# isi-vista/VistaOCR

Measured on AMD Instinct MI355X. Metric: line-images/sec (train, batch 32, 30x600 grey), higher is better.
Workload: dtype f32 (the LSTM's large GEMMs as bf16x6 products: fp32 operands split exactly into three bf16 planes, six bf16 MFMAs per fp32 product, fp32 accumulate; VOCR_LSTM_GEMM=f32 restores the f32-MFMA kernels); 1 GPU; configs[1]: 32 synthetic 1x30x600 grey lines per GPU, 20 labels/line, V=96, 3xBiLSTM-512, train() = H2D of the batch + fwd+CTC+bwd+allreduce+clamp+Adam, loss returned as a float; widths=600 .. 600 px, mean 600, conv_dtype=fp32, global_batch=32, parallelism=dp1, ranks_seen=1, backend=none, per_rank_rng=seed 1234 + 1000*rank after an identical init

## Files before the change

### include/vocr.h

```cpp
#ifndef VOCR_H
#define VOCR_H
#include <stddef.h>
#include <stdint.h>

#ifdef __cplusplus
extern "C" {
#endif

#define VOCR_OK          0
#define VOCR_EINVAL     -1
#define VOCR_ELAUNCH    -2
#define VOCR_ENODEVICE  -3
#define VOCR_ECOMM      -4


const char* vocr_last_error(void);
#define VOCR_ABI_VERSION 5
int  vocr_abi_version(void);
int  vocr_profile_range_push(const char* name);
int  vocr_profile_range_pop(void);
int  vocr_device_count(void);

int vocr_conv3x3_pack_weights(const float* w, float* wpack_fwd, float* wpack_dgrad, int cout, int cin, void* stream);
int vocr_conv3x3_fwd(const float* x, const float* wpack, const float* bias, float* y,
// ... 22 lines not shown
int vocr_conv3x3_wgrad_f16(const float* x, const float* dy, float* dw, void* workspace,
                           int n, int cin, int h, int w, int cout, void* stream);
int vocr_conv3x3_h16_supported(int cin, int cout);
int vocr_conv3x3_h16_plan(int n, int cin, int h, int w, int cout);
int vocr_conv3x3_h16_fwd(const void* x16, const void* wpack, const float* bias, float* y,
                         int n, int cin, int h, int w, int cout, void* stream);
int vocr_f16_padded_row(int w);
int vocr_f32_to_f16_layouts(const float* x, void* nhwc, void* nchwp, int n, int c, int h, int w, void* stream);
int vocr_conv3x3_wgrad_h16_supported(int cin, int cout);
size_t vocr_conv3x3_wgrad_h16_workspace_bytes(int n, int cin, int h, int w, int cout);
int vocr_conv3x3_wgrad_h16(const void* x16p, const void* dy16p, float* dw, void* workspace,
                           int n, int cin, int h, int w, int cout, void* stream);
size_t vocr_channel_sum_workspace_bytes(int n, int c, int hw);
int vocr_channel_sum(const float* x, float* out, int n, int c, int hw, void* workspace, void* stream);

size_t vocr_bn_workspace_bytes(int n, int c, int hw);
int vocr_bn_train_stats(const float* y, int n, int c, int hw, float eps, float momentum,
                        float* mean, float* invstd, float* running_mean, float* running_var,
                        int64_t* num_batches_tracked, float* xhat_sum, void* workspace, void* stream);
int vocr_bn_eval_stats(const float* running_mean, const float* running_var, int c, float eps,
                       float* mean, float* invstd, void* stream);
int vocr_bn_relu_apply(const float* y, const float* mean, const float* invstd, const float* gamma,
                       const float* beta, float* out, int n, int c, int hw, void* stream);
int vocr_bn_train_relu_apply(const float* y, const float* gamma, const float* beta, float* out, int n, int c, int hw, float eps,
                             float momentum, float* mean, float* invstd, float* running_mean, float* running_var,
                             int64_t* num_batches_tracked, float* xhat_sum, void* workspace, void* stream);
int vocr_bn_train_relu_fracpool2x2_fwd(const float* y, const float* gamma, const float* beta, const float* samples, float* out,
                                       int32_t* idx, int n, int c, int h, int w, int oh, int ow, float eps, float momentum,
                                       float* mean, float* invstd, float* running_mean, float* running_var,
                                       int64_t* num_batches_tracked, float* xhat_sum, void* workspace, void* stream);
int vocr_bn_relu_bwd(const float* da, const float* y, const float* mean, const float* invstd,
                     const float* gamma, const float* beta, const float* xhat_sum, float* dy, float* dgamma, float* dbeta,
                     float* dconv_bias, int n, int c, int hw, void* workspace, void* stream);

int vocr_fracpool2x2_fwd(const float* x, const float* samples, float* out, int32_t* idx,
                         int n, int c, int h, int w, int oh, int ow, void* stream);
int vocr_bn_relu_fracpool2x2_fwd(const float* y, const float* mean, const float* invstd, const float* gamma,
                                 const float* beta, const float* samples, float* out, int32_t* idx,
                                 int n, int c, int h, int w, int oh, int ow, void* stream);
int vocr_bn_relu_fracpool2x2_bwd_supported(int h, int w, int oh, int ow);
int vocr_bn_relu_fracpool2x2_bwd(const float* dout, const int32_t* idx, const float* samples, const float* y,
                                 const float* mean, const float* invstd, const float* gamma, const float* beta,
                                 const float* xhat_sum, float* dy, float* dgamma, float* dbeta, float* dconv_bias,
                                 int n, int c, int h, int w, int oh, int ow, void* workspace, void* stream);
int vocr_fracpool2x2_bwd(const float* dout, const int32_t* idx, float* dx,
                         int n, int c, int h, int w, int oh, int ow, void* stream);

int vocr_relu_maxpool2_fwd(const float* x, float* out, int32_t* idx, int n, int c, int h, int w, void* stream);
int vocr_relu_maxpool2_bwd(const float* dout, const float* out, const int32_t* idx, float* dx,
                           int n, int c, int h, int w, void* stream);

size_t vocr_gemm_workspace_bytes(int m, int n, int k, int has_bias_or_relu);
int vocr_gemm(int transa, int transb, int m, int n, int k,
              const float* a, int lda, const float* b, int ldb, float* c, int ldc,
              const float* bias, int relu, int accumulate, void* workspace, size_t workspace_bytes, void* stream);
#define VOCR_GEMM_PLAN_INTS 12
int vocr_gemm_plan(int transa, int transb, int m, int n, int k, int lda, int ldb, int ldc, int aligned, int has_bias_or_relu,
                   int accumulate, size_t workspace_bytes, int nprob, int nseg, int tiles_only, int* plan);
size_t vocr_gemm_pair_workspace_bytes(int m, int n, int k, int mode);
int vocr_gemm_pair(int mode, int transa, int transb, int m, int n, int k, const float* a0, const float* a1, int lda,
                   const float* b0, const float* b1, int ldb, float* c0, float* c1, int ldc, const float* bias0, const float* bias1,
                   int relu, void* workspace, size_t workspace_bytes, void* stream);
size_t vocr_colsum_workspace_bytes(int m, int n);
int vocr_colsum(const float* x, float* out, int m, int n, void* workspace, void* stream);
int vocr_relu_bwd(const float* dy, const float* out, float* dz, size_t count, void* stream);
int vocr_bchw_to_wbch(const float* x, float* out, int b, int c, int h, int w, void* stream);
// ... 172 lines not shown
```

### vistaocr_amd/_lib.py

```python
import ctypes
import os
from ctypes import c_char_p, c_float, c_int, c_size_t, c_uint32, c_uint64, c_void_p

_HERE = os.path.dirname(os.path.abspath(__file__))
LIB_PATH = os.path.join(_HERE, "csrc", "libvocr.so")

P, I, F, Z, U64, U32 = c_void_p, c_int, c_float, c_size_t, c_uint64, c_uint32

SIGNATURES = {
    "vocr_last_error": (c_char_p, []),
    "vocr_abi_version": (I, []),
    "vocr_device_count": (I, []),
    "vocr_profile_range_push": (I, [c_char_p]),
    "vocr_profile_range_pop": (I, []),
    "vocr_conv3x3_pack_weights": (I, [P, P, P, I, I, P]),
    "vocr_conv3x3_fwd": (I, [P, P, P, P, I, I, I, I, I, P]),
    "vocr_conv3x3_wgrad_workspace_bytes": (Z, [I, I, I, I, I]),
    "vocr_conv3x3_wgrad": (I, [P, P, P, P, I, I, I, I, I, P]),
    "vocr_conv3x3_wino_supported": (I, [I, I]),
    "vocr_conv3x3_wino_pack_floats": (Z, [I, I]),
    "vocr_conv3x3_wino_pack_weights": (I, [P, P, P, I, I, P]),
    "vocr_conv3x3_wino_fwd": (I, [P, P, P, P, I, I, I, I, I, P]),
    "vocr_conv3x3_wino_plan": (I, [I, I, I, I, I]),
    "vocr_conv3x3_wgrad_wino_workspace_bytes": (Z, [I, I, I, I, I]),
    "vocr_conv3x3_wgrad_wino": (I, [P, P, P, P, I, I, I, I, I, P]),
    "vocr_conv3x3_f16_pack_bytes": (Z, [I, I, I]),
    "vocr_conv3x3_f16_pack_weights": (I, [P, P, P, I, I, P]),
    "vocr_conv3x3_f16_fwd": (I, [P, P, P, P, I, I, I, I, I, P]),
    "vocr_conv3x3_wgrad_f16": (I, [P, P, P, P, I, I, I, I, I, P]),
    "vocr_conv3x3_c1_fwd": (I, [P, P, P, P, I, I, I, I, I, P]),
    "vocr_conv3x3_c1_wgrad_workspace_bytes": (Z, [I, I, I]),
    "vocr_conv3x3_c1_wgrad": (I, [P, P, P, P, P, I, I, I, I, P]),
    "vocr_conv3x3_h16_supported": (I, [I, I]),
    "vocr_conv3x3_h16_plan": (I, [I, I, I, I, I]),
    "vocr_conv3x3_h16_fwd": (I, [P, P, P, P, I, I, I, I, I, P]),
    "vocr_f16_padded_row": (I, [I]),
    "vocr_f32_to_f16_layouts": (I, [P, P, P, I, I, I, I, P]),
    "vocr_conv3x3_wgrad_h16_supported": (I, [I, I]),
    "vocr_conv3x3_wgrad_h16_workspace_bytes": (Z, [I, I, I, I, I]),
    "vocr_conv3x3_wgrad_h16": (I, [P, P, P, P, I, I, I, I, I, P]),
    "vocr_channel_sum_workspace_bytes": (Z, [I, I, I]),
    "vocr_channel_sum": (I, [P, P, I, I, I, P, P]),
    "vocr_bn_workspace_bytes": (Z, [I, I, I]),
    "vocr_bn_train_stats": (I, [P, I, I, I, F, F, P, P, P, P, P, P, P, P]),
    "vocr_bn_eval_stats": (I, [P, P, I, F, P, P, P]),
    "vocr_bn_relu_apply": (I, [P, P, P, P, P, P, I, I, I, P]),
    "vocr_bn_train_relu_apply": (I, [P, P, P, P, I, I, I, F, F, P, P, P, P, P, P, P, P]),
    "vocr_bn_train_relu_fracpool2x2_fwd": (I, [P, P, P, P, P, P, I, I, I, I, I, I, F, F, P, P, P, P, P, P, P, P]),
    "vocr_bn_relu_bwd": (I, [P, P, P, P, P, P, P, P, P, P, P, I, I, I, P, P]),
    "vocr_bn_relu_fracpool2x2_bwd_supported": (I, [I, I, I, I]),
    "vocr_bn_relu_fracpool2x2_bwd": (I, [P] * 13 + [I] * 6 + [P, P]),
    "vocr_fracpool2x2_fwd": (I, [P, P, P, P, I, I, I, I, I, I, P]),
    "vocr_bn_relu_fracpool2x2_fwd": (I, [P, P, P, P, P, P, P, P, I, I, I, I, I, I, P]),
    "vocr_fracpool2x2_bwd": (I, [P, P, P, I, I, I, I, I, I, P]),
    "vocr_relu_maxpool2_fwd": (I, [P, P, P, I, I, I, I, P]),
    "vocr_relu_maxpool2_bwd": (I, [P, P, P, P, I, I, I, I, P]),
    "vocr_gemm_workspace_bytes": (Z, [I, I, I, I]),
    "vocr_gemm": (I, [I, I, I, I, I, P, I, P, I, P, I, P, I, I, P, Z, P]),
    "vocr_gemm_plan": (I, [I, I, I, I, I, I, I, I, I, I, I, Z, I, I, I, P]),
    "vocr_gemm_pair_workspace_bytes": (Z, [I, I, I, I]),
    "vocr_gemm_pair": (I, [I, I, I, I, I, I, P, P, I, P, P, I, P, P, I, P, P, I, P, Z, P]),
    "vocr_gemm_x6_planes_bytes": (Z, [I, I]),
    "vocr_gemm_x6_split": (I, [P, P, I, I, P, ctypes.c_long, I, I, I, P, P]),
    "vocr_gemm_x6_workspace_bytes": (Z, [I, I, I]),
    "vocr_gemm_x6_plan": (I, [I, I, I, I, I, I, I, P]),
    "vocr_gemm_x6": (I, [P, I, I, I, I, P, I, I, I, I, I, I, I, P, P, I, I, I, P, P, I, P, P]),
    "vocr_gemm_x6_two_views": (I, [P, I, I, I, P, I, I, I, I, I, I, I, I, I, I, I, I, P, P, I, P, P]),
    "vocr_gemm_h3_two_views": (I, [P, I, I, I, P, I, I, I, I, I, I, I, I, I, I, I, I, P, P, I, P, P]),
    "vocr_gemm_h3_planes_bytes": (Z, [I, I]),
    "vocr_gemm_h3_split": (I, [P, P, I, I, P, ctypes.c_long, I, I, I, ctypes.c_float, P, P]),
    "vocr_gemm_h3": (I, [P, I, I, I, I, P, I, I, I, I, I, I, I, P, P, I, I, I, P, P, I, P, P]),
    "vocr_colsum_workspace_bytes": (Z, [I, I]),
    "vocr_colsum": (I, [P, P, I, I, P, P]),
    "vocr_relu_bwd": (I, [P, P, P, Z, P]),
    "vocr_bchw_to_wbch": (I, [P, P, I, I, I, I, P]),
    "vocr_wbch_to_bchw": (I, [P, P, I, I, I, I, P]),
    "vocr_mul": (I, [P, P, P, Z, P]),
    "vocr_add": (I, [P, P, P, Z, P]),
    "vocr_scale_dev": (I, [P, P, P, Z, P]),
    "vocr_dropout_fwd": (I, [P, P, P, Z, F, U64, P]),
    "vocr_dropout_mask": (I, [P, Z, F, U64, P]),
    "vocr_lstm_workspace_bytes": (Z, [I, I, I]),
# ... 138 lines not shown
```

### vistaocr_amd/build.py

```python
import hashlib
import json
import os
import shutil
import subprocess
import sys
from concurrent.futures import ThreadPoolExecutor

CSRC = os.path.join(os.path.dirname(os.path.abspath(__file__)), "csrc")
SOURCES = ["gemm.hip", "gemm_dma.hip", "gemm_x6.hip", "conv.hip", "conv_wino.hip", "conv_f16.hip", "bn_pool.hip", "lstm.hip", "ctc.hip", "ctc_beam.hip", "ctc_word_beam.hip", "ctc_align.hip", "ctc_edit.hip", "ctc_nbest.hip", "ctc_entropy.hip", "ctc_keyword.hip", "ctc_grammar.hip", "ctc_grammar_beam.hip", "edit_distance.hip", "augment.hip", "misc.cpp", "comm.cpp"]
HEADERS = [os.path.join(CSRC, "vocr_common.h"), os.path.join(CSRC, "conv_tail.h"), os.path.join(CSRC, "gemm_dma.h"),
           os.path.join(CSRC, "ctc_math.h"), os.path.join(CSRC, "ctc_beam_common.h"), os.path.join(CSRC, "ctc_align_common.h"),
           os.path.join(CSRC, "ctc_lattice.h"),
           os.path.join(CSRC, "..", "..", "include", "vocr.h")]
LIB = os.path.join(CSRC, "libvocr.so")
STAMP = os.path.join(CSRC, "build", "libvocr.stamp")
ARCH = "gfx950"
FLAGS = ["-O3", "--offload-arch=" + ARCH, "-fPIC", "-std=c++17", "-Wno-pass-failed"]
_REPORT = {"built": False, "reason": "not asked"}


def _hipcc():
    for cand in (shutil.which("hipcc"), "/opt/rocm/bin/hipcc"):
        if cand and os.path.exists(cand):
            return cand
    return None


def _tree_hash():
    h = hashlib.sha256()
    for path in [os.path.join(CSRC, s) for s in SOURCES] + HEADERS:
        h.update(os.path.basename(path).encode() + b"\0")
        with open(path, "rb") as f:
            h.update(f.read())
    h.update(" ".join(FLAGS).encode())
    return h.hexdigest()


def tree_hash():
    return _tree_hash()


def _compiler_id(hipcc):
    if not hipcc:
# ... 90 lines not shown
```

### vistaocr_amd/csrc/bn_pool.hip

```cpp
#include "vocr_common.h"

namespace {

constexpr int BN_CHUNK_ELEMS = 16384;

__host__ __device__ inline int bn_nchunk(long per_channel) {
    long n = (per_channel + BN_CHUNK_ELEMS - 1) / BN_CHUNK_ELEMS;
    return (int)(n < 1 ? 1 : (n > 512 ? 512 : n));
}

__device__ __forceinline__ long chan_addr(long e, int c, int C, long HW) {
    const long n = e / HW, r = e - n * HW;
    return (n * C + c) * HW + r;
}

struct ChanWalk {
    long n;
    long r;
    __device__ __forceinline__ ChanWalk(long e, long HW) : n(e / HW), r(e - (e / HW) * HW) {}
    __device__ __forceinline__ long addr(int c, int C, long HW) const { return (n * C + c) * HW + r; }
    __device__ __forceinline__ void advance(long step, long HW) {
        r += step;
        while (r >= HW) { r -= HW; ++n; }
    }
};

__device__ __forceinline__ void block_reduce2(double& a, double& b, double* red) {
    a = wave_sum_d(a);
    b = wave_sum_d(b);
    const int wave = threadIdx.x >> 6;
    if ((threadIdx.x & 63) == 0) { red[wave * 2] = a; red[wave * 2 + 1] = b; }
    __syncthreads();
    a = (red[0] + red[2]) + (red[4] + red[6]);
// ... 806 lines not shown
        pool_bwd_lds_kernel<8192><<<(unsigned)(n * c), 512, 0, s>>>(dout, idx, dx, (int)in_plane, oh * ow);
    } else if (use_lds && in_plane <= 18432) {
        pool_bwd_lds_kernel<18432><<<(unsigned)(n * c), 512, 0, s>>>(dout, idx, dx, (int)in_plane, oh * ow);
    } else if (use_lds && in_plane <= 36864) {
        pool_bwd_lds_kernel<36864><<<(unsigned)(n * c), 512, 0, s>>>(dout, idx, dx, (int)in_plane, oh * ow);
    } else {
        if (hipMemsetAsync(dx, 0, (size_t)n * c * in_plane * sizeof(float), s) != hipSuccess) {
            vocr_set_error("vocr_fracpool2x2_bwd: memset failed");
            return VOCR_ELAUNCH;
        }
        pool_bwd_scatter_kernel<<<plane_grid((long)n * c, (long)oh * ow), 256, 0, s>>>(dout, idx, dx, in_plane, oh * ow);
    }
    VOCR_CHECK_LAUNCH("vocr_fracpool2x2_bwd");
    return VOCR_OK;
}

extern "C" int vocr_relu_maxpool2_fwd(const float* x, float* out, int32_t* idx, int n, int c, int h, int w, void* stream) {
    VOCR_CHECK_ARG(x && out && idx && n > 0 && c > 0 && h >= 2 && w >= 2 && (long)n * c <= 65535, "vocr_relu_maxpool2_fwd: bad argument");
    const int oh = h / 2, ow = w / 2;
    relu_maxpool2_fwd_kernel<<<plane_grid((long)n * c, (long)oh * ow), 256, 0, (hipStream_t)stream>>>(x, out, idx, h, w, oh, ow);
    VOCR_CHECK_LAUNCH("vocr_relu_maxpool2_fwd");
    return VOCR_OK;
}

extern "C" int vocr_relu_maxpool2_bwd(const float* dout, const float* out, const int32_t* idx, float* dx, int n, int c,
                                      int h, int w, void* stream) {
    VOCR_CHECK_ARG(dout && out && idx && dx && n > 0 && c > 0 && (long)n * c <= 65535, "vocr_relu_maxpool2_bwd: bad argument");
    const int oh = h / 2, ow = w / 2;
    relu_maxpool2_bwd_kernel<<<plane_grid((long)n * c, (long)oh * ow), 256, 0, (hipStream_t)stream>>>(dout, out, idx, dx,
                                                                                                  (long)h * w, oh * ow);
    VOCR_CHECK_LAUNCH("vocr_relu_maxpool2_bwd");
    return VOCR_OK;
}
```

### vistaocr_amd/csrc/conv.hip

```cpp
#include "vocr_common.h"
#include "conv_tail.h"

namespace {

constexpr int SEGW = 32;
constexpr int CI_C = 8;
constexpr int KC = CI_C * 9;
constexpr int PROW = SEGW + 2;
constexpr int PCI = 3 * PROW;
constexpr int PSEG = CI_C * PCI;

__global__ void pack_weights_kernel(const float* __restrict__ w, float* __restrict__ pf, float* __restrict__ pd,
                                    int cout, int cin) {
    const int i = blockIdx.x * blockDim.x + threadIdx.x;
    const int total = cout * cin * 9;
    if (i >= total) return;
    const int tap = i % 9, ci = (i / 9) % cin, co = i / (9 * cin);
    const float v = w[i];
    if (pf) pf[(long)(ci * 9 + tap) * cout + co] = v;
    if (pd) pd[(long)(co * 9 + (8 - tap)) * cin + ci] = v;
}

struct SegGeom { int FS, RW, RR, per_img, nseg; };

__host__ __device__ inline SegGeom seg_geom(int N, int H, int W) {
    SegGeom g;
    g.FS = W / SEGW;
    g.RW = W % SEGW;
    g.RR = g.RW ? (PROW / (g.RW + 2)) : 1;
    if (g.RR > H) g.RR = H;
    g.per_img = H * g.FS + (g.RW ? (H + g.RR - 1) / g.RR : 0);
    g.nseg = N * g.per_img;
    return g;
}
// ... 1270 lines not shown
    const int QW = (W + 3) >> 2;
    const int q = blockIdx.x * 256 + threadIdx.x;
    if (q >= H * QW) return;
    const int h = q / QW, w0 = (q % QW) * 4;
    const float* xi = x + (long)n * H * W;
    float win[3][6];
#pragma unroll
    for (int kh = 0; kh < 3; ++kh) {
        const int hh = h + kh - 1;
        const bool rok = hh >= 0 && hh < H;
        const float* row = xi + (long)(rok ? hh : 0) * W;
#pragma unroll
        for (int j = 0; j < 6; ++j) {
            const int ww = w0 - 1 + j;
            float v = (rok && ww >= 0 && ww < W) ? row[ww] : 0.f;
            if (round_f16) v = (float)(_Float16)v;
            win[kh][j] = v;
        }
    }
    float* yo = y + ((long)n * Cout * H + h) * W + w0;
    const long cstride = (long)H * W;
    const bool full = w0 + 3 < W && ((((uintptr_t)yo) | ((uintptr_t)(cstride * 4))) & 15) == 0;
    for (int co = 0; co < Cout; ++co) {
        float k[9];
#pragma unroll
        for (int t = 0; t < 9; ++t) {
            k[t] = w[co * 9 + t];
            if (round_f16) k[t] = (float)(_Float16)k[t];
        }
        const float b = bias ? bias[co] : 0.f;
        float o[4];
#pragma unroll
        for (int p = 0; p < 4; ++p) {
            float a = 0.f;
#pragma unroll
            for (int kh = 0; kh < 3; ++kh)
#pragma unroll
                for (int kw = 0; kw < 3; ++kw) a = __builtin_fmaf(win[kh][p + kw], k[kh * 3 + kw], a);
            o[p] = a + b;
        }
        float* d = yo + co * cstride;
        if (full) {
            *(f32x4*)d = (f32x4){o[0], o[1], o[2], o[3]};
        } else {
#pragma unroll
            for (int p = 0; p < 4; ++p)
                if (w0 + p < W) d[p] = o[p];
        }
    }
}

__global__ __launch_bounds__(256) void conv3x3_c1_wgrad_kernel(const float* __restrict__ x, const float* __restrict__ dy,
                                                               float* __restrict__ part, int N, int H, int W, int Cout, int rows_per_split) {
    __shared__ float red[40][257];
    const int tid = threadIdx.x;
    const int cg = blockIdx.x, split = blockIdx.y;
    const int co0 = cg * 4;
    const int nco = min(4, Cout - co0);
    const long HW = (long)H * W;
    const int r0 = split * rows_per_split, r1 = min(N * H, r0 + rows_per_split);
    float acc[4][10];
#pragma unroll
    for (int c = 0; c < 4; ++c)
#pragma unroll
        for (int t = 0; t < 10; ++t) acc[c][t] = 0.f;
    const int QW = (W + 3) >> 2;
    const bool vec = (W & 3) == 0 && ((((uintptr_t)x) | ((uintptr_t)dy)) & 15) == 0;
    for (long q = (long)r0 * QW + tid; q < (long)r1 * QW; q += 256) {
        const int r = (int)(q / QW), w0 = (int)(q % QW) * 4;
        const int n = r / H, h = r % H;
        const float* xi = x + (long)n * HW;
        const float* dyb = dy + ((long)n * Cout + co0) * HW + (long)h * W + w0;
// ... 106 lines not shown
```

### vistaocr_amd/ops.py

```python
import math

import torch

from . import _lib
from ._lib import call, prof_range


def _stream():
    return torch.cuda.current_stream().cuda_stream


def _ranged(name):
    def deco(fn):
        if not _lib.ROCTX:
            return fn

        def wrapped(*a, **k):
            with prof_range(name):
                return fn(*a, **k)
        wrapped.__name__ = fn.__name__
        wrapped.__doc__ = fn.__doc__
        return wrapped
    return deco

# ... 187 lines not shown
            ev = torch.cuda.Event()
            ev.record(side)
            prep.pack_events[w.data_ptr()] = ev
        for (w_hh_f, b_ih_f, b_hh_f, w_hh_r, b_ih_r, b_hh_r) in lstm_layers:
            H4 = b_ih_f.numel()
            bsum = torch.empty(2, H4, dtype=torch.float32, device=b_ih_f.device)
            call("vocr_add", _p(b_ih_f), _p(b_hh_f), _p(bsum[0]), H4, _stream())
            call("vocr_add", _p(b_ih_r), _p(b_hh_r), _p(bsum[1]), H4, _stream())
            wt = (transpose2d(w_hh_f), transpose2d(w_hh_r)) if with_transposes else (None, None)
            prep.lstm[w_hh_f.data_ptr()] = (bsum, wt[0], wt[1])
            made.extend(t for t in (bsum,) + wt if t is not None)
        for (w_ih_f, w_ih_r) in x6_layers:
            if w_ih_f.shape[1] >= 512:
                prep.x6w[w_ih_f.data_ptr()] = x6_weight_planes(w_ih_f, w_ih_r, with_transposes)
                made.extend(t for t in prep.x6w[w_ih_f.data_ptr()] if t is not None)
        for (w_ih_f, w_ih_r) in follow_layers:
            prep.xpack[w_ih_f.data_ptr()] = lstm_xproj_pack(w_ih_f, w_ih_r)
            made.append(prep.xpack[w_ih_f.data_ptr()])
        prep.event = torch.cuda.Event()
        prep.event.record(side)
    for t in made:
        t.record_stream(main)
    return prep


_BN_FUSED_FINAL = _exp("VOCR_BN_FUSED_FINAL", "1") == "1"
_WINO = _exp("VOCR_CONV_WINO", "1") == "1"
_WINO_WGRAD = _exp("VOCR_WGRAD_WINO", "1") == "1"


_WINO_MIN_CIN = int(_exp("VOCR_CONV_WINO_MIN_CIN", "1"))


def _wino_ok(cin, cout):
    return _WINO and cin >= _WINO_MIN_CIN and cout % 4 == 0


def conv3x3_pack(weight):
    cout, cin = weight.shape[0], weight.shape[1]
    dev = weight.device
    wf, wd = _wino_ok(cin, cout), _wino_ok(cout, cin)
    lib = _lib.load()
    rows_f = lib.vocr_conv3x3_wino_pack_floats(cout, cin) // (cout * cin)
    rows_d = lib.vocr_conv3x3_wino_pack_floats(cin, cout) // (cout * cin)
    pf = torch.empty(cin * (rows_f if wf else 9), cout, dtype=torch.float32, device=dev)
    pd = torch.empty(cout * (rows_d if wd else 9), cin, dtype=torch.float32, device=dev)
    if wf or wd:
        call("vocr_conv3x3_wino_pack_weights", _p(weight), _p(pf) if wf else None, _p(pd) if wd else None, cout, cin, _stream())
    if not (wf and wd):
        call("vocr_conv3x3_pack_weights", _p(weight), None if wf else _p(pf), None if wd else _p(pd), cout, cin, _stream())
    return pf, pd


def conv3x3_pack_f16(weight):
    cout, cin = weight.shape[0], weight.shape[1]
    lib = _lib.load()
    pf = torch.empty(lib.vocr_conv3x3_f16_pack_bytes(cout, cin, 0) // 2, dtype=torch.float16, device=weight.device)
    pd = torch.empty(lib.vocr_conv3x3_f16_pack_bytes(cout, cin, 1) // 2, dtype=torch.float16, device=weight.device)
    call("vocr_conv3x3_f16_pack_weights", _p(weight), _p(pf), _p(pd), cout, cin, _stream())
    return pf, pd


def f16_layouts(x, want_nhwc=True, want_nchwp=False):
    n, c, h, w = x.shape
    nhwc = torch.empty(n, c // 16, h, w, 16, dtype=torch.float16, device=x.device) if want_nhwc else None
    nchwp = torch.empty(n, c, h, _lib.load().vocr_f16_padded_row(w), dtype=torch.float16, device=x.device) if want_nchwp else None
# ... 63 lines not shown
        ws = _ws(lib.vocr_conv3x3_wgrad_h16_workspace_bytes(n, cin, h, w, cout), x.device)
        call("vocr_conv3x3_wgrad_h16", _p(x16p), _p(dy16p), _p(dw), _p(ws), n, cin, h, w, cout, _stream())
        return dw
    if _WINO_WGRAD and cin >= 4 and n * max(cin, cout) * h * w < (1 << 29):
        ws = _ws(lib.vocr_conv3x3_wgrad_wino_workspace_bytes(n, cin, h, w, cout), x.device)
        call("vocr_conv3x3_wgrad_wino", _p(x), _p(dy), _p(dw), _p(ws), n, cin, h, w, cout, _stream())
        return dw
    ws = _ws(lib.vocr_conv3x3_wgrad_workspace_bytes(n, cin, h, w, cout), x.device)
    call("vocr_conv3x3_wgrad_f16" if f16 else "vocr_conv3x3_wgrad", _p(x), _p(dy), _p(dw), _p(ws), n, cin, h, w, cout, _stream())
    return dw


def channel_sum(x, out=None):
    n, c, h, w = x.shape
    out = out if out is not None else torch.empty(c, dtype=torch.float32, device=x.device)
    nb = _lib.load().vocr_channel_sum_workspace_bytes(n, c, h * w)
    ws = _ws(nb, x.device) if nb else None
    call("vocr_channel_sum", _p(x), _p(out), n, c, h * w, _p(ws), _stream())
    return out


class ConvBnReluFn(torch.autograd.Function):

    @staticmethod
    def forward(ctx, x, weight, bias, gamma, beta, running_mean, running_var, training, eps, momentum, f16=False,
                pool_samples=None, pool_oh=0, pool_ow=0, num_batches_tracked=None, prep=None):
        _need_gpu(x, weight, bias, gamma, beta, running_mean, running_var)
        x = _f32c(x)
        n, cin, h, w = x.shape
        cout = weight.shape[0]
        lib = _lib.load()
        ctx.f16 = bool(f16)
        x16p = None
        if cin == 1 and not ctx.needs_input_grad[0]:
            pf = pd = None
            y = conv3x3_c1_forward(x, weight, bias, ctx.f16)
        elif ctx.f16:
            if prep is not None and weight.data_ptr() in prep.packs:
                prep.wait_pack(weight.data_ptr())
                pf, pd = prep.packs[weight.data_ptr()]
            else:
                pf, pd = conv3x3_pack_f16(weight)
            x_nhwc = None
            if h16_takes(n, cin, h, w, cout):
                x_nhwc, x16p = f16_layouts(x, True, bool(training) and wgrad_f16_layouts_ok(cin, cout))
            y = conv3x3_forward_f16(x, pf, bias, cout, x_nhwc)
        else:
            if prep is not None and weight.data_ptr() in prep.packs:
                prep.wait_pack(weight.data_ptr())
                pf, pd = prep.packs[weight.data_ptr()]
            else:
                pf, pd = conv3x3_pack(weight)
            y = conv3x3_forward(x, pf, bias, cout)
        mean = torch.empty(cout, dtype=torch.float32, device=x.device)
        invstd = torch.empty(cout, dtype=torch.float32, device=x.device)
        xhat_sum = None
        fused_final = training and _BN_FUSED_FINAL
        ws = None
        if training:
            ws = _ws(lib.vocr_bn_workspace_bytes(n, cout, h * w), x.device)
            xhat_sum = torch.empty(cout, dtype=torch.float32, device=x.device)
            if not fused_final:
                call("vocr_bn_train_stats", _p(y), n, cout, h * w, eps, momentum, _p(mean), _p(invstd), _p(running_mean),
                     _p(running_var), _p(num_batches_tracked), _p(xhat_sum), _p(ws), _stream())
        else:
            call("vocr_bn_eval_stats", _p(running_mean), _p(running_var), cout, eps, _p(mean), _p(invstd), _stream())
        ctx.pool = None
        idx = samples = None
        if pool_samples is not None:
            samples = _f32c(pool_samples)
            if tuple(samples.shape) != (n, cout, 2):
                raise RuntimeError("fractional pool samples must have shape (N, C, 2)")
            out = torch.empty(n, cout, pool_oh, pool_ow, dtype=torch.float32, device=x.device)
            idx = torch.empty(n, cout, pool_oh, pool_ow, dtype=torch.int32, device=x.device)
            if fused_final:
                call("vocr_bn_train_relu_fracpool2x2_fwd", _p(y), _p(gamma), _p(beta), _p(samples), _p(out), _p(idx), n, cout, h, w, pool_oh, pool_ow,
                     eps, momentum, _p(mean), _p(invstd), _p(running_mean), _p(running_var), _p(num_batches_tracked), _p(xhat_sum), _p(ws), _stream())
            else:
                call("vocr_bn_relu_fracpool2x2_fwd", _p(y), _p(mean), _p(invstd), _p(gamma), _p(beta), _p(samples), _p(out), _p(idx),
                     n, cout, h, w, pool_oh, pool_ow, _stream())
            ctx.pool = (pool_oh, pool_ow)
        else:
            out = torch.empty_like(y)
            if fused_final:
                call("vocr_bn_train_relu_apply", _p(y), _p(gamma), _p(beta), _p(out), n, cout, h * w, eps, momentum, _p(mean), _p(invstd),
                     _p(running_mean), _p(running_var), _p(num_batches_tracked), _p(xhat_sum), _p(ws), _stream())
            else:
                call("vocr_bn_relu_apply", _p(y), _p(mean), _p(invstd), _p(gamma), _p(beta), _p(out), n, cout, h * w, _stream())
        ctx.training = training
        ctx.prefs = (weight, bias, gamma, beta)
        ctx.save_for_backward(x, y, mean, invstd, gamma, beta, pd, idx, samples, xhat_sum, x16p)
        return out

    @staticmethod
    @_ranged("bwd.conv_bn_relu")
    def backward(ctx, da):
        if not ctx.training:
            raise RuntimeError("vistaocr_amd: backward through eval-mode BatchNorm is not part of the reference path")
        x, y, mean, invstd, gamma, beta, pd, idx, samples, xhat_sum, x16p = ctx.saved_tensors
        da = _f32c(da)
        n, cin, h, w = x.shape
        cout = y.shape[1]
        lib = _lib.load()
        fused_pool_bwd = False
        if ctx.pool is not None:
            oh, ow = ctx.pool
            fused_pool_bwd = bool(lib.vocr_bn_relu_fracpool2x2_bwd_supported(h, w, oh, ow)) and _exp("VOCR_POOL_BWD_FUSED", "1") == "1"
            if not fused_pool_bwd:
                dfull = torch.empty(n, cout, h, w, dtype=torch.float32, device=da.device)
                call("vocr_fracpool2x2_bwd", _p(da), _p(idx), _p(dfull), n, cout, h, w, oh, ow, _stream())
                da = dfull
        dy = torch.empty_like(y)
        sinks = _sinks(ctx.prefs)
        if sinks is not None:
            dw, dbias, dgamma, dbeta = sinks
        else:
            dw = None
            dgamma = torch.empty_like(gamma)
            dbeta = torch.empty_like(beta)
            dbias = torch.empty(cout, dtype=torch.float32, device=x.device)
        ws = _ws(lib.vocr_bn_workspace_bytes(n, cout, h * w), x.device)
        if fused_pool_bwd:
            call("vocr_bn_relu_fracpool2x2_bwd", _p(da), _p(idx), _p(samples), _p(y), _p(mean), _p(invstd), _p(gamma), _p(beta),
                 _p(xhat_sum), _p(dy), _p(dgamma), _p(dbeta), _p(dbias), n, cout, h, w, oh, ow, _p(ws), _stream())
        else:
            call("vocr_bn_relu_bwd", _p(da), _p(y), _p(mean), _p(invstd), _p(gamma), _p(beta), _p(xhat_sum), _p(dy), _p(dgamma),
                 _p(dbeta), _p(dbias), n, cout, h * w, _p(ws), _stream())
        dy_nhwc = dy16p = None
        if ctx.f16:
            want_nhwc = bool(ctx.needs_input_grad[0]) and h16_takes(dy.shape[0], cout, dy.shape[2], dy.shape[3], cin)
            if want_nhwc or x16p is not None:
                dy_nhwc, dy16p = f16_layouts(dy, want_nhwc, x16p is not None)
        if sinks is not None and _SIDE_ENABLED and ctx.needs_input_grad[0] and _exp("VOCR_CONV_OVERLAP", "1") == "1":
            side = side_stream()
            side.wait_stream(torch.cuda.current_stream())
            for t_ in (x, dy, x16p, dy16p):
                if t_ is not None:
                    t_.record_stream(side)
            with torch.cuda.stream(side):
                conv3x3_wgrad(x, dy, out=dw, f16=ctx.f16, x16p=x16p, dy16p=dy16p)
            mark_side_pending()
        else:
            dw = conv3x3_wgrad(x, dy, out=dw, f16=ctx.f16, x16p=x16p, dy16p=dy16p)
        dx = None
        if ctx.needs_input_grad[0]:
            dx = conv3x3_forward_f16(dy, pd, None, cin, dy_nhwc) if ctx.f16 else conv3x3_forward(dy, pd, None, cin)
        else:
            join_side_stream()
        if sinks is not None:
            return (dx,) + (None,) * 15
        return (dx, dw, dbias, dgamma, dbeta) + (None,) * 11


class ConvReluPoolFn(torch.autograd.Function):

    @staticmethod
    def forward(ctx, x, weight, bias, f16=False):
        _need_gpu(x, weight, bias)
        x = _f32c(x)
        n, cin, h, w = x.shape
        cout = weight.shape[0]
        ctx.f16 = bool(f16)
        if cin == 1 and not ctx.needs_input_grad[0]:
            pf = pd = None
            y = conv3x3_c1_forward(x, weight, bias, ctx.f16)
        elif ctx.f16:
            pf, pd = conv3x3_pack_f16(weight)
            y = conv3x3_forward_f16(x, pf, bias, cout)
        else:
            pf, pd = conv3x3_pack(weight)
            y = conv3x3_forward(x, pf, bias, cout)
        oh, ow = h // 2, w // 2
        out = torch.empty(n, cout, oh, ow, dtype=torch.float32, device=x.device)
        idx = torch.empty(n, cout, oh, ow, dtype=torch.int32, device=x.device)
        call("vocr_relu_maxpool2_fwd", _p(y), _p(out), _p(idx), n, cout, h, w, _stream())
        ctx.save_for_backward(x, out, idx, pd)
        ctx.prefs = (weight, bias)
        ctx.hw = (h, w)
        return out

    @staticmethod
    @_ranged("bwd.rapid_ds")
    def backward(ctx, dout):
        x, out, idx, pd = ctx.saved_tensors
        dout = _f32c(dout)
# ... 1021 lines not shown
```

Baseline: 2315 line-images/sec.

## Fuse first-layer single-channel conv with BN+ReLU, recomputing conv in backward

```diff
diff --git a/include/vocr.h b/include/vocr.h
--- a/include/vocr.h
+++ b/include/vocr.h
@@ -78,6 +78,15 @@
 int vocr_bn_relu_bwd(const float* da, const float* y, const float* mean, const float* invstd,
                      const float* gamma, const float* beta, const float* xhat_sum, float* dy, float* dgamma, float* dbeta,
                      float* dconv_bias, int n, int c, int hw, void* workspace, void* stream);
+size_t vocr_conv3x3_c1_bn_workspace_bytes(int n, int h, int wd, int cout);
+int vocr_conv3x3_c1_bn_train_relu(const float* x, const float* w, const float* bias, const float* gamma, const float* beta, float* out,
+                                  int n, int h, int wd, int cout, float eps, float momentum, float* mean, float* invstd,
+                                  float* running_mean, float* running_var, int64_t* num_batches_tracked, float* xhat_sum,
+                                  void* workspace, void* stream);
+int vocr_conv3x3_c1_bn_relu_bwd(const float* da, const float* x, const float* w, const float* bias, const float* mean,
+                                const float* invstd, const float* gamma, const float* beta, const float* xhat_sum, float* dw,
+                                float* dgamma, float* dbeta, float* dconv_bias, int n, int h, int wd, int cout, void* workspace,
+                                void* stream);
 
 int vocr_fracpool2x2_fwd(const float* x, const float* samples, float* out, int32_t* idx,
                          int n, int c, int h, int w, int oh, int ow, void* stream);
diff --git a/vistaocr_amd/_lib.py b/vistaocr_amd/_lib.py
--- a/vistaocr_amd/_lib.py
+++ b/vistaocr_amd/_lib.py
@@ -48,6 +48,9 @@
     "vocr_bn_train_relu_apply": (I, [P, P, P, P, I, I, I, F, F, P, P, P, P, P, P, P, P]),
     "vocr_bn_train_relu_fracpool2x2_fwd": (I, [P, P, P, P, P, P, I, I, I, I, I, I, F, F, P, P, P, P, P, P, P, P]),
     "vocr_bn_relu_bwd": (I, [P, P, P, P, P, P, P, P, P, P, P, I, I, I, P, P]),
+    "vocr_conv3x3_c1_bn_workspace_bytes": (Z, [I, I, I, I]),
+    "vocr_conv3x3_c1_bn_train_relu": (I, [P, P, P, P, P, P, I, I, I, I, F, F, P, P, P, P, P, P, P, P]),
+    "vocr_conv3x3_c1_bn_relu_bwd": (I, [P] * 13 + [I, I, I, I, P, P]),
     "vocr_bn_relu_fracpool2x2_bwd_supported": (I, [I, I, I, I]),
     "vocr_bn_relu_fracpool2x2_bwd": (I, [P] * 13 + [I] * 6 + [P, P]),
     "vocr_fracpool2x2_fwd": (I, [P, P, P, P, I, I, I, I, I, I, P]),
diff --git a/vistaocr_amd/build.py b/vistaocr_amd/build.py
--- a/vistaocr_amd/build.py
+++ b/vistaocr_amd/build.py
@@ -8,7 +8,7 @@
 
 CSRC = os.path.join(os.path.dirname(os.path.abspath(__file__)), "csrc")
 SOURCES = ["gemm.hip", "gemm_dma.hip", "gemm_x6.hip", "conv.hip", "conv_wino.hip", "conv_f16.hip", "bn_pool.hip", "lstm.hip", "ctc.hip", "ctc_beam.hip", "ctc_word_beam.hip", "ctc_align.hip", "ctc_edit.hip", "ctc_nbest.hip", "ctc_entropy.hip", "ctc_keyword.hip", "ctc_grammar.hip", "ctc_grammar_beam.hip", "edit_distance.hip", "augment.hip", "misc.cpp", "comm.cpp"]
-HEADERS = [os.path.join(CSRC, "vocr_common.h"), os.path.join(CSRC, "conv_tail.h"), os.path.join(CSRC, "gemm_dma.h"),
+HEADERS = [os.path.join(CSRC, "vocr_common.h"), os.path.join(CSRC, "conv_tail.h"), os.path.join(CSRC, "conv_c1.h"), os.path.join(CSRC, "gemm_dma.h"),
            os.path.join(CSRC, "ctc_math.h"), os.path.join(CSRC, "ctc_beam_common.h"), os.path.join(CSRC, "ctc_align_common.h"),
            os.path.join(CSRC, "ctc_lattice.h"),
            os.path.join(CSRC, "..", "..", "include", "vocr.h")]
diff --git a/vistaocr_amd/csrc/bn_pool.hip b/vistaocr_amd/csrc/bn_pool.hip
--- a/vistaocr_amd/csrc/bn_pool.hip
+++ b/vistaocr_amd/csrc/bn_pool.hip
@@ -1,4 +1,5 @@
 #include "vocr_common.h"
+#include "conv_c1.h"
 
 namespace {
 
@@ -871,3 +872,320 @@
     VOCR_CHECK_LAUNCH("vocr_relu_maxpool2_bwd");
     return VOCR_OK;
 }
+
+namespace {
+
+template <int V, bool ROW>
+__global__ __launch_bounds__(256) void conv3x3_c1_bn_stats_partial_kernel(const float* __restrict__ x, const float* __restrict__ w,
+                                                                          const float* __restrict__ bias, double* __restrict__ part, int N,
+                                                                          int H, int W, int nchunk, long per, int xvec) {
+    __shared__ double red[8];
+    const int c = blockIdx.x, j = blockIdx.y;
+    float flt[9];
+#pragma unroll
+    for (int t = 0; t < 9; ++t) flt[t] = w[c * 9 + t];
+    const float cb = bias ? bias[c] : 0.f;
+    const long HW = (long)H * W, total = (long)N * HW;
+    const long beg = j * per, end = min(total, beg + per);
+    double s = 0.0, q = 0.0;
+    C1Walk wk(beg + (long)threadIdx.x * V, 256 * V, H, W);
+    for (long e = beg + (long)threadIdx.x * V; e < end; e += 256 * V, wk.advance(H, W)) {
+        C1Taps<V, ROW> tp;
+        tp.load(x + (long)wk.n * HW, H, W, wk.h, wk.w, xvec);
+#pragma unroll
+        for (int i = 0; i < V; ++i) {
+            const double y = (double)tp.y(i, flt, cb);
+            s += y;
+            q += y * y;
+        }
+    }
+    block_reduce2(s, q, red);
+    if (threadIdx.x == 0) {
+        part[((long)c * nchunk + j) * 2] = s;
+        part[((long)c * nchunk + j) * 2 + 1] = q;
+    }
+}
+
+template <int V, bool ROW>
+__global__ __launch_bounds__(256) void conv3x3_c1_bn_relu_apply_kernel(const float* __restrict__ x, const float* __restrict__ w,
+                                                                       const float* __restrict__ bias, const float* __restrict__ gamma,
+                                                                       const float* __restrict__ beta, float* __restrict__ out, int C, int H,
+                                                                       int W, BnFusedStats fs, int xvec, int ovec) {
+    typedef typename VecT<V>::type vec;
+    __shared__ double stage[2 * BN_MAX_CHUNKS + 2];
+    const long plane = blockIdx.y;
+    const int c = (int)(plane % C);
+    float mu, is;
+    double s_, q_;
+    combine_partials(fs.part, c, fs.nchunk, stage, s_, q_);
+    bn_train_stats_of(s_, q_, fs.count, fs.eps, fs.momentum, c, blockIdx.x == 0 && plane < C, fs.mean, fs.invstd, fs.rmean, fs.rvar, fs.nbt,
+                      fs.xhat_sum, mu, is);
+    const float g = gamma[c], b = beta[c];
+    float flt[9];
+#pragma unroll
+    for (int t = 0; t < 9; ++t) flt[t] = w[c * 9 + t];
+    const float cb = bias ? bias[c] : 0.f;
+    const long HW = (long)H * W;
+    const float* xi = x + (plane / C) * HW;
+    float* op = out + plane * HW;
+    const long nv = HW / V;
+    const long i0 = (long)blockIdx.x * 256 + threadIdx.x, stride = (long)gridDim.x * 256;
+    C1Walk wk(i0 * V, stride * V, H, W);
+    for (long i = i0; i < nv; i += stride, wk.advance(H, W)) {
+        C1Taps<V, ROW> tp;
+        tp.load(xi, H, W, wk.h, wk.w, xvec);
+        vec o;
+#pragma unroll
+        for (int k = 0; k < V; ++k) {
+            const float v = (tp.y(k, flt, cb) - mu) * is * g + b;
+            vset<V>(o, k, v > 0.f ? v : 0.f);
+        }
+        if (ovec) {
+            *(vec*)(op + i * V) = o;
+        } else {
+#pragma unroll
+            for (int k = 0; k < V; ++k) op[i * V + k] = vget<V>(o, k);
+        }
+    }
+}
+
+template <int V> __device__ __forceinline__ typename VecT<V>::type c1_load_da(const float* __restrict__ da, long a, int dvec) {
+    typename VecT<V>::type v;
+    if (dvec) {
+        v = *(const typename VecT<V>::type*)(da + a);
+    } else {
+#pragma unroll
+        for (int k = 0; k < V; ++k) vset<V>(v, k, da[a + k]);
+    }
+    return v;
+}
+
+template <int V, bool ROW>
+__global__ __launch_bounds__(256) void conv3x3_c1_bn_bwd_partial_kernel(const float* __restrict__ da, const float* __restrict__ x,
+                                                                        const float* __restrict__ w, const float* __restrict__ bias,
+                                                                        const float* __restrict__ mean, const float* __restrict__ invstd,
+                                                                        const float* __restrict__ gamma, const float* __restrict__ beta,
+                                                                        double* __restrict__ part, int N, int C, int H, int W, int nchunk,
+                                                                        long per, int xvec, int dvec) {
+    typedef typename VecT<V>::type vec;
+    __shared__ double red[8];
+    const int c = blockIdx.x, j = blockIdx.y;
+    const float mu = mean[c], is = invstd[c], g = gamma[c], b = beta[c];
+    float flt[9];
+#pragma unroll
+    for (int t = 0; t < 9; ++t) flt[t] = w[c * 9 + t];
+    const float cb = bias ? bias[c] : 0.f;
+    const long HW = (long)H * W, total = (long)N * HW;
+    const long beg = j * per, end = min(total, beg + per);
+    double s1 = 0.0, s2 = 0.0;
+    __builtin_amdgcn_s_setprio(3);
+    constexpr int U = 2;
+    C1Walk wk(beg + (long)threadIdx.x * V, 256 * V, H, W);
+    for (long e = beg + (long)threadIdx.x * V; e < end; e += (long)U * 256 * V) {
+        vec dv[U];
+        bool ok[U];
+        int pn[U], ph[U], pw[U];
+        const int n0 = wk.n, h0 = wk.h, w0 = wk.w;
+#pragma unroll
+        for (int u = 0; u < U; ++u) {
+            ok[u] = e + (long)u * 256 * V < end;
+            pn[u] = ok[u] ? wk.n : n0;
+            ph[u] = ok[u] ? wk.h : h0;
+            pw[u] = ok[u] ? wk.w : w0;
+            dv[u] = c1_load_da<V>(da, ((long)pn[u] * C + c) * HW + (long)ph[u] * W + pw[u], dvec);
+            wk.advance(H, W);
+        }
+#pragma unroll
+        for (int u = 0; u < U; ++u) {
+            C1Taps<V, ROW> tp;
+            tp.load(x + (long)pn[u] * HW, H, W, ph[u], pw[u], xvec);
+            float p1 = 0.f, p2 = 0.f;
+#pragma unroll
+            for (int k = 0; k < V; ++k) {
+                const float xh = (tp.y(k, flt, cb) - mu) * is;
+                const float o = xh * g + b;
+                const float dz = o > 0.f ? vget<V>(dv[u], k) : 0.f;
+                p1 += dz;
+                p2 += dz * xh;
+            }
+            if (ok[u]) {
+                s1 += (double)p1;
+                s2 += (double)p2;
+            }
+        }
+    }
+    block_reduce2(s1, s2, red);
+    if (threadIdx.x == 0) {
+        part[((long)c * nchunk + j) * 2] = s1;
+        part[((long)c * nchunk + j) * 2 + 1] = s2;
+    }
+}
+
+template <int V, bool ROW>
+__global__ __launch_bounds__(256) void conv3x3_c1_bn_bwd_wgrad_kernel(const float* __restrict__ da, const float* __restrict__ x,
+                                                                      const float* __restrict__ w, const float* __restrict__ bias,
+                                                                      const float* __restrict__ mean, const float* __restrict__ invstd,
+                                                                      const float* __restrict__ gamma, const float* __restrict__ beta,
+                                                                      float* __restrict__ dgamma, float* __restrict__ dbeta,
+                                                                      float* __restrict__ dconv_bias, const float* __restrict__ xhat_sum,
+                                                                      const double* __restrict__ part, double* __restrict__ wpart, int N, int C,
+                                                                      int H, int W, int nchunk, long per, float inv_count, double inv_count_d,
+                                                                      int xvec, int dvec) {
+    typedef typename VecT<V>::type vec;
+    __shared__ double stage[2 * BN_MAX_CHUNKS + 2];
+    __shared__ double red[4][9];
+    const int c = blockIdx.x, j = blockIdx.y;
+    const float mu = mean[c], is = invstd[c], g = gamma[c], b = beta[c];
+    double s1, s2;
+    combine_partials(part, c, nchunk, stage, s1, s2);
+    const float dbeta_c = (float)s1, dgamma_c = (float)s2;
+    if (j == 0 && threadIdx.x == 0) {
+        dbeta[c] = dbeta_c;
+        dgamma[c] = dgamma_c;
+        if (dconv_bias) dconv_bias[c] = xhat_sum ? (float)(-(double)g * (double)is * (s2 * inv_count_d) * (double)xhat_sum[c]) : 0.f;
+    }
+    const float k1 = dbeta_c * inv_count, k2 = dgamma_c * inv_count, gs = g * is;
+    float flt[9];
+#pragma unroll
+    for (int t = 0; t < 9; ++t) flt[t] = w[c * 9 + t];
+    const float cb = bias ? bias[c] : 0.f;
+    const long HW = (long)H * W, total = (long)N * HW;
+    const long beg = j * per, end = min(total, beg + per);
+    double acc[9];
+#pragma unroll
+    for (int t = 0; t < 9; ++t) acc[t] = 0.0;
+    __builtin_amdgcn_s_setprio(3);
+    constexpr int U = 2;
+    C1Walk wk(beg + (long)threadIdx.x * V, 256 * V, H, W);
+    for (long e = beg + (long)threadIdx.x * V; e < end; e += (long)U * 256 * V) {
+        vec dv[U];
+        bool ok[U];
+        int pn[U], ph[U], pw[U];
+        const int n0 = wk.n, h0 = wk.h, w0 = wk.w;
+#pragma unroll
+        for (int u = 0; u < U; ++u) {
+            ok[u] = e + (long)u * 256 * V < end;
+            pn[u] = ok[u] ? wk.n : n0;
+            ph[u] = ok[u] ? wk.h : h0;
+            pw[u] = ok[u] ? wk.w : w0;
+            dv[u] = c1_load_da<V>(da, ((long)pn[u] * C + c) * HW + (long)ph[u] * W + pw[u], dvec);
+            wk.advance(H, W);
+        }
+#pragma unroll
+        for (int u = 0; u < U; ++u) {
+            C1Taps<V, ROW> tp;
+            tp.load(x + (long)pn[u] * HW, H, W, ph[u], pw[u], xvec);
+            float a9[9];
+#pragma unroll
+            for (int t = 0; t < 9; ++t) a9[t] = 0.f;
+#pragma unroll
+            for (int k = 0; k < V; ++k) {
+                const float xh = (tp.y(k, flt, cb) - mu) * is;
+                const float ov = xh * g + b;
+                const float dz = ov > 0.f ? vget<V>(dv[u], k) : 0.f;
+                const float dy = gs * (dz - k1 - xh * k2);
+#pragma unroll
+                for (int kh = 0; kh < 3; ++kh)
+#pragma unroll
+                    for (int kw = 0; kw < 3; ++kw) a9[kh * 3 + kw] = __builtin_fmaf(dy, tp.tap(k, kh, kw), a9[kh * 3 + kw]);
+            }
+            if (ok[u]) {
+#pragma unroll
+                for (int t = 0; t < 9; ++t) acc[t] += (double)a9[t];
+            }
+        }
+    }
+    const int wave = threadIdx.x >> 6, lane = threadIdx.x & 63;
+#pragma unroll
+    for (int t = 0; t < 9; ++t) {
+        const double v = wave_sum_d(acc[t]);
+        if (lane == 0) red[wave][t] = v;
+    }
+    __syncthreads();
+    if (threadIdx.x < 9) {
+        const int t = threadIdx.x;
+        wpart[((long)c * nchunk + j) * 9 + t] = (red[0][t] + red[1][t]) + (red[2][t] + red[3][t]);
+    }
+}
+
+__global__ __launch_bounds__(64) void conv3x3_c1_bn_wgrad_final_kernel(const double* __restrict__ wpart, float* __restrict__ dw, int nchunk) {
+    __shared__ double stage[BN_MAX_CHUNKS];
+    const int c = blockIdx.x / 9, t = blockIdx.x % 9;
+    for (int j = threadIdx.x; j < nchunk; j += 64) stage[j] = wpart[((long)c * nchunk + j) * 9 + t];
+    __syncthreads();
+    if (threadIdx.x == 0) {
+        double a = 0.0;
+        for (int j = 0; j < nchunk; ++j) a += stage[j];
+        dw[blockIdx.x] = (float)a;
+    }
+}
+
+inline int c1_bn_vec(long hw) { return hw % 4 == 0 ? 4 : (hw % 2 == 0 ? 2 : 1); }
+inline int c1_aligned(const void* p, int V) { return ((uintptr_t)p & (uintptr_t)(V * 4 - 1)) == 0; }
+
+}
+
+#define VOCR_C1_BN_LAUNCH(kernel, grid, block, s, ...)                                                   \
+    do {                                                                                                 \
+        if (V == 4 && row) kernel<4, true><<<grid, block, 0, s>>>(__VA_ARGS__);                          \
+        else if (V == 4) kernel<4, false><<<grid, block, 0, s>>>(__VA_ARGS__);                           \
+        else if (V == 2 && row) kernel<2, true><<<grid, block, 0, s>>>(__VA_ARGS__);                     \
+        else if (V == 2) kernel<2, false><<<grid, block, 0, s>>>(__VA_ARGS__);                           \
+        else kernel<1, true><<<grid, block, 0, s>>>(__VA_ARGS__);                                        \
+    } while (0)
+
+extern "C" size_t vocr_conv3x3_c1_bn_workspace_bytes(int n, int h, int w, int cout) {
+    if (n <= 0 || h <= 0 || w <= 0 || cout <= 0) return 0;
+    return (size_t)cout * bn_nchunk((long)n * h * w) * (2 + 9) * sizeof(double);
+}
+
+extern "C" int vocr_conv3x3_c1_bn_train_relu(const float* x, const float* w, const float* bias, const float* gamma, const float* beta, float* out,
+                                             int n, int h, int wd, int cout, float eps, float momentum, float* mean, float* invstd,
+                                             float* running_mean, float* running_var, int64_t* num_batches_tracked, float* xhat_sum,
+                                             void* workspace, void* stream) {
+    VOCR_CHECK_ARG(x && w && gamma && beta && out && mean && invstd && workspace, "vocr_conv3x3_c1_bn_train_relu: null pointer");
+    VOCR_CHECK_ARG(n > 0 && h > 0 && wd > 0 && cout > 0 && (long)n * cout <= 65535 && (long)h * wd < (1L << 31) && cout <= 65535,
+                   "vocr_conv3x3_c1_bn_train_relu: bad shape n=%d h=%d w=%d cout=%d", n, h, wd, cout);
+    hipStream_t s = (hipStream_t)stream;
+    const long hw = (long)h * wd;
+    const int V = c1_bn_vec(hw);
+    const bool row = wd % V == 0;
+    const int xvec = row && c1_aligned(x, V), ovec = c1_aligned(out, V);
+    const int nchunk = bn_nchunk((long)n * hw);
+    const long per = chunk_len((long)n * hw, nchunk);
+    VOCR_C1_BN_LAUNCH(conv3x3_c1_bn_stats_partial_kernel, dim3(cout, nchunk), 256, s, x, w, bias, (double*)workspace, n, h, wd, nchunk, per, xvec);
+    VOCR_CHECK_LAUNCH("vocr_conv3x3_c1_bn_train_relu(partial)");
+    const BnFusedStats fs = {(const double*)workspace, nchunk, (long)n * hw, eps, momentum, mean, invstd, running_mean, running_var, xhat_sum,
+                             (long long*)num_batches_tracked};
+    const dim3 grid = plane_grid((long)n * cout, hw / V);
+    VOCR_C1_BN_LAUNCH(conv3x3_c1_bn_relu_apply_kernel, grid, 256, s, x, w, bias, gamma, beta, out, cout, h, wd, fs, xvec, ovec);
+    VOCR_CHECK_LAUNCH("vocr_conv3x3_c1_bn_train_relu(apply)");
+    return VOCR_OK;
+}
+
+extern "C" int vocr_conv3x3_c1_bn_relu_bwd(const float* da, const float* x, const float* w, const float* bias, const float* mean,
+                                           const float* invstd, const float* gamma, const float* beta, const float* xhat_sum, float* dw,
+                                           float* dgamma, float* dbeta, float* dconv_bias, int n, int h, int wd, int cout, void* workspace,
+                                           void* stream) {
+    VOCR_CHECK_ARG(da && x && w && mean && invstd && gamma && beta && dw && dgamma && dbeta && workspace, "vocr_conv3x3_c1_bn_relu_bwd: null pointer");
+    VOCR_CHECK_ARG(n > 0 && h > 0 && wd > 0 && cout > 0 && (long)n * cout <= 65535 && (long)h * wd < (1L << 31) && cout <= 65535,
+                   "vocr_conv3x3_c1_bn_relu_bwd: bad shape n=%d h=%d w=%d cout=%d", n, h, wd, cout);
+    hipStream_t s = (hipStream_t)stream;
+    const long hw = (long)h * wd;
+    const int V = c1_bn_vec(hw);
+    const bool row = wd % V == 0;
+    const int xvec = row && c1_aligned(x, V), dvec = c1_aligned(da, V);
+    const int nchunk = bn_nchunk((long)n * hw);
+    const long per = chunk_len((long)n * hw, nchunk);
+    double* part = (double*)workspace;
+    double* wpart = part + (size_t)cout * nchunk * 2;
+    VOCR_C1_BN_LAUNCH(conv3x3_c1_bn_bwd_partial_kernel, dim3(cout, nchunk), 256, s, da, x, w, bias, mean, invstd, gamma, beta, part, n, cout, h, wd,
+                      nchunk, per, xvec, dvec);
+    VOCR_CHECK_LAUNCH("vocr_conv3x3_c1_bn_relu_bwd(partial)");
+    VOCR_C1_BN_LAUNCH(conv3x3_c1_bn_bwd_wgrad_kernel, dim3(cout, nchunk), 256, s, da, x, w, bias, mean, invstd, gamma, beta, dgamma, dbeta, dconv_bias,
+                      xhat_sum, part, wpart, n, cout, h, wd, nchunk, per, 1.0f / (float)((long)n * hw), 1.0 / (double)((long)n * hw), xvec, dvec);
+    VOCR_CHECK_LAUNCH("vocr_conv3x3_c1_bn_relu_bwd(wgrad)");
+    conv3x3_c1_bn_wgrad_final_kernel<<<cout * 9, 64, 0, s>>>(wpart, dw, nchunk);
+    VOCR_CHECK_LAUNCH("vocr_conv3x3_c1_bn_relu_bwd(final)");
+    return VOCR_OK;
+}
diff --git a/vistaocr_amd/csrc/conv.hip b/vistaocr_amd/csrc/conv.hip
--- a/vistaocr_amd/csrc/conv.hip
+++ b/vistaocr_amd/csrc/conv.hip
@@ -1,5 +1,6 @@
 #include "vocr_common.h"
 #include "conv_tail.h"
+#include "conv_c1.h"
 
 namespace {
 
@@ -1336,12 +1337,12 @@
         float o[4];
 #pragma unroll
         for (int p = 0; p < 4; ++p) {
-            float a = 0.f;
+            float t[9];
 #pragma unroll
             for (int kh = 0; kh < 3; ++kh)
 #pragma unroll
-                for (int kw = 0; kw < 3; ++kw) a = __builtin_fmaf(win[kh][p + kw], k[kh * 3 + kw], a);
-            o[p] = a + b;
+                for (int kw = 0; kw < 3; ++kw) t[kh * 3 + kw] = win[kh][p + kw];
+            o[p] = conv3x3_c1_y(t, k, b);
         }
         float* d = yo + co * cstride;
         if (full) {
diff --git a/vistaocr_amd/csrc/conv_c1.h b/vistaocr_amd/csrc/conv_c1.h
--- /dev/null
+++ b/vistaocr_amd/csrc/conv_c1.h
@@ -0,0 +1,90 @@
+#pragma once
+#include "vocr_common.h"
+
+__device__ __forceinline__ float conv3x3_c1_y(const float (&t)[9], const float (&k)[9], float b) {
+#pragma clang fp contract(off)
+    float a = 0.f;
+#pragma unroll
+    for (int i = 0; i < 9; ++i) a = __builtin_fmaf(t[i], k[i], a);
+    return a + b;
+}
+
+struct C1Walk {
+    int n, h, w;
+    int dh, dw;
+    __device__ __forceinline__ C1Walk(long e, long step, int H, int W) {
+        const long HW = (long)H * W;
+        n = (int)(e / HW);
+        const int r = (int)(e - n * HW);
+        h = r / W;
+        w = r - h * W;
+        dh = (int)(step / W);
+        dw = (int)(step - (long)dh * W);
+    }
+    __device__ __forceinline__ void advance(int H, int W) {
+        w += dw;
+        h += dh;
+        if (w >= W) { w -= W; ++h; }
+        while (h >= H) { h -= H; ++n; }
+    }
+};
+
+template <int V, bool ROW> struct C1Taps {
+    float v[ROW ? 3 : 3 * V][ROW ? V + 2 : 3];
+    __device__ __forceinline__ void load(const float* __restrict__ xi, int H, int W, int h, int w, bool vec) {
+        typedef float vecf __attribute__((ext_vector_type(V > 1 ? V : 2)));
+        if constexpr (ROW) {
+#pragma unroll
+            for (int kh = 0; kh < 3; ++kh) {
+                const int hh = h + kh - 1;
+                const bool rok = hh >= 0 && hh < H;
+                const float* row = xi + (long)(rok ? hh : 0) * W;
+                if (V > 1 && vec) {
+                    vecf q;
+#pragma unroll
+                    for (int j = 0; j < V; ++j) q[j] = 0.f;
+                    if (rok) q = *(const vecf*)(row + w);
+#pragma unroll
+                    for (int j = 0; j < V; ++j) v[kh][1 + j] = q[j];
+                    v[kh][0] = (rok && w > 0) ? row[w - 1] : 0.f;
+                    v[kh][V + 1] = (rok && w + V < W) ? row[w + V] : 0.f;
+                } else {
+#pragma unroll
+                    for (int j = 0; j < V + 2; ++j) {
+                        const int ww = w - 1 + j;
+                        v[kh][j] = (rok && ww >= 0 && ww < W) ? row[ww] : 0.f;
+                    }
+                }
+            }
+        } else {
+            int hi = h, wi = w;
+#pragma unroll
+            for (int i = 0; i < V; ++i) {
+#pragma unroll
+                for (int kh = 0; kh < 3; ++kh) {
+                    const int hh = hi + kh - 1;
+                    const bool rok = hh >= 0 && hh < H;
+                    const float* row = xi + (long)(rok ? hh : 0) * W;
+#pragma unroll
+                    for (int kw = 0; kw < 3; ++kw) {
+                        const int ww = wi + kw - 1;
+                        v[3 * i + kh][kw] = (rok && ww >= 0 && ww < W) ? row[ww] : 0.f;
+                    }
+                }
+                if (++wi >= W) { wi = 0; ++hi; }
+            }
+        }
+    }
+    __device__ __forceinline__ float tap(int i, int kh, int kw) const {
+        if constexpr (ROW) return v[kh][i + kw];
+        else return v[3 * i + kh][kw];
+    }
+    __device__ __forceinline__ float y(int i, const float (&k)[9], float b) const {
+        float t[9];
+#pragma unroll
+        for (int kh = 0; kh < 3; ++kh)
+#pragma unroll
+            for (int kw = 0; kw < 3; ++kw) t[kh * 3 + kw] = tap(i, kh, kw);
+        return conv3x3_c1_y(t, k, b);
+    }
+};
diff --git a/vistaocr_amd/ops.py b/vistaocr_amd/ops.py
--- a/vistaocr_amd/ops.py
+++ b/vistaocr_amd/ops.py
@@ -243,6 +243,11 @@
 _WINO_MIN_CIN = int(_exp("VOCR_CONV_WINO_MIN_CIN", "1"))
 
 
+def c1_fused_takes(cin, weight, f16, training, pooled, needs_input_grad):
+    return (cin == 1 and tuple(weight.shape[2:]) == (3, 3) and weight.dtype == torch.float32 and not f16 and bool(training) and not pooled
+            and not needs_input_grad and _BN_FUSED_FINAL and _exp("VOCR_C1_FUSED", "1") == "1")
+
+
 def _wino_ok(cin, cout):
     return _WINO and cin >= _WINO_MIN_CIN and cout % 4 == 0
 
@@ -372,6 +377,18 @@
         lib = _lib.load()
         ctx.f16 = bool(f16)
         x16p = None
+        ctx.c1_fused = c1_fused_takes(cin, weight, ctx.f16, training, pool_samples is not None, ctx.needs_input_grad[0])
+        if ctx.c1_fused:
+            mean, invstd, xhat_sum = (torch.empty(cout, dtype=torch.float32, device=x.device) for _ in range(3))
+            out = torch.empty(n, cout, h, w, dtype=torch.float32, device=x.device)
+            ws = _ws(lib.vocr_conv3x3_c1_bn_workspace_bytes(n, h, w, cout), x.device)
+            call("vocr_conv3x3_c1_bn_train_relu", _p(x), _p(weight), _p(bias), _p(gamma), _p(beta), _p(out), n, h, w, cout, eps, momentum,
+                 _p(mean), _p(invstd), _p(running_mean), _p(running_var), _p(num_batches_tracked), _p(xhat_sum), _p(ws), _stream())
+            ctx.pool = None
+            ctx.training = training
+            ctx.prefs = (weight, bias, gamma, beta)
+            ctx.save_for_backward(x, None, mean, invstd, gamma, beta, None, None, None, xhat_sum, None, weight, bias)
+            return out
         if cin == 1 and not ctx.needs_input_grad[0]:
             pf = pd = None
             y = conv3x3_c1_forward(x, weight, bias, ctx.f16)
@@ -437,6 +454,8 @@
     def backward(ctx, da):
         if not ctx.training:
             raise RuntimeError("vistaocr_amd: backward through eval-mode BatchNorm is not part of the reference path")
+        if ctx.c1_fused:
+            return ConvBnReluFn._backward_c1_fused(ctx, da)
         x, y, mean, invstd, gamma, beta, pd, idx, samples, xhat_sum, x16p = ctx.saved_tensors
         da = _f32c(da)
         n, cin, h, w = x.shape
@@ -491,6 +510,28 @@
             return (dx,) + (None,) * 15
         return (dx, dw, dbias, dgamma, dbeta) + (None,) * 11
 
+    @staticmethod
+    def _backward_c1_fused(ctx, da):
+        x, _, mean, invstd, gamma, beta, _, _, _, xhat_sum, _, weight, bias = ctx.saved_tensors
+        da = _f32c(da)
+        n, _, h, w = x.shape
+        cout = weight.shape[0]
+        sinks = _sinks(ctx.prefs)
+        if sinks is not None:
+            dw, dbias, dgamma, dbeta = sinks
+        else:
+            dw = torch.empty_like(weight)
+            dgamma = torch.empty_like(gamma)
+            dbeta = torch.empty_like(beta)
+            dbias = torch.empty(cout, dtype=torch.float32, device=x.device)
+        ws = _ws(_lib.load().vocr_conv3x3_c1_bn_workspace_bytes(n, h, w, cout), x.device)
+        call("vocr_conv3x3_c1_bn_relu_bwd", _p(da), _p(x), _p(weight), _p(bias), _p(mean), _p(invstd), _p(gamma), _p(beta), _p(xhat_sum),
+             _p(dw), _p(dgamma), _p(dbeta), _p(dbias), n, h, w, cout, _p(ws), _stream())
+        join_side_stream()
+        if sinks is not None:
+            return (None,) * 16
+        return (None, dw, dbias, dgamma, dbeta) + (None,) * 11
+
 
 class ConvReluPoolFn(torch.autograd.Function):
 
```

Result: no change. 2308 line-images/sec, median of 2 (-0.3%).
